# showlab/EgoVLP

Measured on AMD Instinct MI355X. Metric: clip-pairs/sec (whole node), 4f/224^2 ViT-B + 32-tok text, B=32/GPU, train step (fwd+gather+EgoNCE+bwd+AdamW), higher is better.
Workload: dtype fp16 (every Linear and both attentions of the video blocks, forward and backward) + bf16 (patch embedding, text tower, heads) MFMA operands, fp32 accumulate

## Files before the change

egovlp_amd/_lib.py:

```python
import ctypes as C
import os

import torch

_HERE = os.path.dirname(os.path.abspath(__file__))
LIB_PATH = os.environ.get("EGOVLP_HIP_LIB", os.path.join(_HERE, "libegovlp_hip.so"))

c_p = C.c_void_p
i32 = C.c_int32
i64 = C.c_int64
f32 = C.c_float
u64 = C.c_uint64


class GemmDesc(C.Structure):
    _fields_ = [
        ("a_hi", c_p), ("a_lo", c_p), ("lda", i64),
        ("b_hi", c_p), ("b_lo", c_p), ("ldb", i64),
        ("M", i32), ("N", i32), ("K", i32), ("passes", i32),
        ("alpha", f32), ("act", i32),
        ("bias", c_p),
        ("residual", c_p), ("ldr", i64),
        ("aux_in", c_p), ("aux_out", c_p), ("ldaux", i64),
        ("out_f32", c_p), ("ldo", i64),
# ... 71 lines not shown
    "egv_egonce_work_floats": (i64, [i32, i32]),
    "egv_sim_matrix_fwd": (i32, [c_p, c_p, i32, i32, i32, f32, c_p, c_p, c_p, c_p, c_p]),
    "egv_sim_matrix_bwd": (i32, [c_p, c_p, c_p, c_p, i32, i32, i32, f32, c_p, c_p, c_p]),
    "egv_egonce_from_sim": (i32, [c_p, c_p, c_p, i32, f32, i32, i32, c_p, c_p, c_p, c_p]),
    "egv_maxmargin_fwd_bwd": (i32, [c_p, c_p, i32, f32, i32, c_p, c_p, c_p]),
    "egv_maxmargin_head_fwd_bwd": (i32, [c_p, c_p, c_p, i32, i32, f32, i32, f32, c_p, c_p, c_p, c_p, c_p, c_p]),
    "egv_maxmargin_head_work_floats": (i64, [i32, i32]),
    "egv_cls_head_fwd": (i32, [c_p, i64, c_p, c_p, i32, i32, i32, c_p, i64, c_p]),
    "egv_cls_head_loss_bwd": (i32, [c_p, i64, i32, i32, i32, i32, i32, i32, c_p, i64, c_p, i32, c_p, c_p, c_p, c_p, i64, c_p, c_p, c_p]),
    "egv_cls_eval_update": (i32, [c_p, i64, i32, i32, i32, i32, i32, i32, i32, i32, c_p, c_p]),
    "egv_dual_softmax": (i32, [c_p, i32, i32, f32, c_p, c_p, c_p]),
    "egv_rank_scores": (i32, [c_p, i64, i32, c_p, i32, i64, i32, i32, i32, c_p, c_p, c_p, c_p]),
    "egv_rank_scores_work_bytes": (i64, [i32, i32]),
    "egv_cross_entropy_fwd_bwd": (i32, [c_p, i64, c_p, i32, i32, i64, c_p, c_p, i64, c_p]),
    "egv_adamw_multi": (i32, [i32, c_p, c_p, c_p, c_p, c_p, c_p, c_p, f32, f32, f32, f32, f32, i32, i32, f32, c_p, c_p]),
    "egv_grad_accumulate_multi": (i32, [i32, c_p, c_p, c_p, c_p]),
    "egv_grad_pack_bf16": (i32, [i32, c_p, c_p, c_p, c_p, f32, c_p]),
    "egv_grad_unpack_bf16": (i32, [i32, c_p, c_p, c_p, c_p, c_p]),
    "egv_slice_sum_bf16": (i32, [c_p, i32, i64, c_p, c_p]),
    "egv_relu_split": (i32, [c_p, i64, i32, i32, c_p, c_p, i64, c_p]),
    "egv_version": (i32, []),
    "egv_abi_check": (i32, [i32, i64, i64, i64, i64]),
    "egv_split_f32_multi_t16": (i32, [i32, c_p, c_p, c_p, c_p, c_p, c_p, c_p, c_p, c_p, c_p, c_p, c_p, c_p]),
    "egv_layernorm_bwd_fmt": (i32, [c_p, c_p, c_p, i64, c_p, i64, c_p, c_p, c_p, i32, i32, c_p, c_p, c_p, i64, c_p, c_p, i32, c_p, c_p, c_p, c_p]),
    "egv_layernorm_bwd_partial": (i32, [c_p, c_p, c_p, i64, c_p, i64, c_p, c_p, c_p, i32, i32, c_p, c_p, c_p, i64, c_p, c_p, i32, c_p, c_p, c_p, c_p]),
    "egv_layernorm_bwd_reduce": (i32, [i32, c_p, i32, i32, c_p, c_p, c_p]),
    "egv_splitk_reduce_multi": (i32, [i32, c_p, c_p, c_p, c_p, c_p, c_p, c_p]),
    "egv_grad_nonfinite_multi": (i32, [i32, c_p, c_p, c_p, c_p]),
    "egv_loss_scale_update": (i32, [c_p, c_p, f32, f32, f32, i32, i32, f32, f32, i32, f32, i32, c_p]),
    "egv_split_f32_multi": (i32, [i32, c_p, c_p, c_p, c_p, c_p, c_p, c_p, c_p, c_p, c_p, c_p, c_p]),
# ... 54 lines not shown
```

egovlp_amd/csrc/adamw.hip:

```cpp
#include "common.h"
#include "egovlp_hip.h"

namespace {

constexpr int MAX_T = 48;
constexpr int CHUNK = 16384;

struct AdamTable {
  float* p[MAX_T];
  const float* g[MAX_T];
  float* m[MAX_T];
  float* v[MAX_T];
  bf16_t* wh[MAX_T];
  bf16_t* wl[MAX_T];
  long numel[MAX_T];
  int blk_start[MAX_T + 1];
  int count;
};

__global__ __launch_bounds__(256) void adamw_kernel(const AdamTable t, float lr, float b1, float b2, float eps, float wd,
                                                    float step_size, float grad_scale, const float* __restrict__ hyper) {
  if (hyper) {
    if (hyper[3] != 0.f) return;
    lr = hyper[0];
    step_size = hyper[1];
    grad_scale = hyper[2];
  }
  int ti = 0;
  while (ti + 1 < t.count && (int)blockIdx.x >= t.blk_start[ti + 1]) ++ti;
  const long base = (long)((int)blockIdx.x - t.blk_start[ti]) * CHUNK;
  const long n = t.numel[ti];
  float* __restrict__ p = t.p[ti];
  const float* __restrict__ g = t.g[ti];
  float* __restrict__ m = t.m[ti];
  float* __restrict__ v = t.v[ti];
  bf16_t* wh = t.wh[ti];
  bf16_t* wl = t.wl[ti];
  const long end = min(n, base + CHUNK);
  const bool vec = ((n & 3) == 0) && (((((size_t)p) | ((size_t)g) | ((size_t)m) | ((size_t)v)) & 15) == 0) &&
                   (!wh || (((size_t)wh) & 7) == 0) && (!wl || (((size_t)wl) & 7) == 0);
  if (vec) {
    for (long i = base + threadIdx.x * 4; i < end; i += 256 * 4) {
      f32x4_t pv = egv_load<EGV_NT_ADAMW_LD, f32x4_t>(p + i), gv = egv_load<EGV_NT_ADAMW_LD, f32x4_t>(g + i),
               mv = egv_load<EGV_NT_ADAMW_LD, f32x4_t>(m + i), vv = egv_load<EGV_NT_ADAMW_LD, f32x4_t>(v + i);
      bf16_t h[4], l[4];
#pragma unroll
      for (int e = 0; e < 4; ++e) {
        const float ge = gv[e] * grad_scale;
        mv[e] = mv[e] * b1 + (1.0f - b1) * ge;
        vv[e] = vv[e] * b2 + (1.0f - b2) * ge * ge;
        const float denom = sqrtf(vv[e]) + eps;
        pv[e] = pv[e] - step_size * (mv[e] / denom);
        if (wd > 0.f) pv[e] = pv[e] - lr * wd * pv[e];
        split_bf16(pv[e], h[e], l[e]);
      }
      egv_store<EGV_NT_ADAMW_ST>(p + i, pv);
      egv_store<EGV_NT_ADAMW_ST>(m + i, mv);
      egv_store<EGV_NT_ADAMW_ST>(v + i, vv);
      if (wh) *(u32x2_t*)(wh + i) = (u32x2_t){pack2(h[0], h[1]), pack2(h[2], h[3])};
      if (wl) *(u32x2_t*)(wl + i) = (u32x2_t){pack2(l[0], l[1]), pack2(l[2], l[3])};
    }
  } else {
    for (long i = base + threadIdx.x; i < end; i += 256) {
      const float ge = g[i] * grad_scale;
      const float me = m[i] * b1 + (1.0f - b1) * ge;
      const float ve = v[i] * b2 + (1.0f - b2) * ge * ge;
      float pe = p[i] - step_size * (me / (sqrtf(ve) + eps));
      if (wd > 0.f) pe = pe - lr * wd * pe;
      p[i] = pe;
      m[i] = me;
      v[i] = ve;
      bf16_t h, l;
      split_bf16(pe, h, l);
      if (wh) wh[i] = h;
      if (wl) wl[i] = l;
    }
  }
}

constexpr int NF_MAX_T = 96;
struct NonfiniteTable {
  const float* g[NF_MAX_T];
  long numel[NF_MAX_T];
  int blk_start[NF_MAX_T + 1];
  int count;
};
__global__ __launch_bounds__(256) void grad_nonfinite_kernel(const NonfiniteTable t, int* __restrict__ state) {
  int ti = 0;
  while (ti + 1 < t.count && (int)blockIdx.x >= t.blk_start[ti + 1]) ++ti;
  const long base = (long)((int)blockIdx.x - t.blk_start[ti]) * (4 * CHUNK);
// ... 217 lines not shown
    if (!p[i] || !g[i] || !m[i] || !v[i]) return EGV_ERR_ARG;
    if (nt == MAX_T) {
      const int rc = flush();
      if (rc) return rc;
    }
    t.p[nt] = p[i]; t.g[nt] = g[i]; t.m[nt] = m[i]; t.v[nt] = v[i];
    t.wh[nt] = w_hi ? w_hi[i] : nullptr;
    t.wl[nt] = w_lo ? w_lo[i] : nullptr;
    t.numel[nt] = numel[i];
    t.blk_start[nt] = nb;
    nb += (int)((numel[i] + CHUNK - 1) / CHUNK);
    ++nt;
  }
  return flush();
}
```

egovlp_amd/csrc/gemm_nt.hip:

```cpp
#include "common.h"
#include "egovlp_hip.h"

namespace {

constexpr int BM = 128, BN = 128, BK = 32;
constexpr int PLANE_BYTES = BM * BK * 2;

struct Frag4 {
  bf16x8_t v[4];
};

__device__ __forceinline__ int swz_g(int x) { return (0x78 >> (2 * x)) & 3; }

__device__ __forceinline__ void glds16(const void* g, char* lds_wave_base) {
  __builtin_amdgcn_global_load_lds((const __attribute__((address_space(1))) void*)g,
                                   (__attribute__((address_space(3))) void*)lds_wave_base, 16, 0, 0);
}

__device__ __forceinline__ void nt_epilogue4(const egv_gemm_desc& p, f32x4_t v, int m, int n) {
  if (p.alpha != 1.0f) v *= p.alpha;
  if (p.bias) v += *(const f32x4_t*)(p.bias + n);
  if (p.act == EGV_ACT_GELU) {
    if (p.aux_out) *(f32x4_t*)(p.aux_out + (long)m * p.ldaux + n) = v;
#pragma unroll
// ... 126 lines not shown
    if (m >= p.M) continue;
#pragma unroll
    for (int j = 0; j < 4; ++j) {
      const int n = n0 + wn * 64 + j * 16 + ln;
      if (n >= p.N) continue;
      f32x4_t v = acc[i][j];
      if (ksplit > 1) {
        *(f32x4_t*)(p.partial + ((long)z * p.M + m) * p.N + n) = v;
        continue;
      }
      nt_epilogue4(p, v, m, n);
    }
  }
}

__global__ __launch_bounds__(256) void splitk_reduce_kernel(const float* __restrict__ partial, float* __restrict__ out,
                                                            long mn, int ksplit, int accumulate,
                                                            const float* __restrict__ partial2, float* __restrict__ out2,
                                                            long n2, int blocks1) {
  if ((int)blockIdx.x >= blocks1) {
    partial = partial2;
    out = out2;
    mn = n2;
    accumulate = 0;
  }
  const long i4 = ((long)((int)blockIdx.x >= blocks1 ? (int)blockIdx.x - blocks1 : (int)blockIdx.x) * blockDim.x + threadIdx.x) * 4;
  if (i4 >= mn) return;
  f32x4_t s = egv_load<EGV_NT_REDUCE_LD, f32x4_t>(partial + i4);
  for (int z = 1; z < ksplit; ++z) s += egv_load<EGV_NT_REDUCE_LD, f32x4_t>(partial + (long)z * mn + i4);
  if (accumulate) s += *(const f32x4_t*)(out + i4);
  egv_store<EGV_NT_WGRAD>(out + i4, s);
}

constexpr int RED_MAX_T = 8;
struct ReduceTable {
  const float* partial[RED_MAX_T];
  float* out[RED_MAX_T];
  float* colsum[RED_MAX_T];
  long mn[RED_MAX_T];
  int m[RED_MAX_T], ks[RED_MAX_T];
  int blk_start[RED_MAX_T + 1];
  int blocks1[RED_MAX_T];
  int count;
};
__global__ __launch_bounds__(256) void splitk_reduce_multi_kernel(const ReduceTable t) {
  int e = 0;
  while (e + 1 < t.count && (int)blockIdx.x >= t.blk_start[e + 1]) ++e;
  const int local = (int)blockIdx.x - t.blk_start[e];
  const int ks = t.ks[e];
  const float* partial = t.partial[e];
  float* out = t.out[e];
  long mn = t.mn[e];
  long i4;
  if (local >= t.blocks1[e]) {
    partial += (long)ks * mn;
    out = t.colsum[e];
    mn = t.m[e];
    i4 = ((long)(local - t.blocks1[e]) * 256 + threadIdx.x) * 4;
  } else {
    i4 = ((long)local * 256 + threadIdx.x) * 4;
  }
  if (i4 >= mn) return;
  f32x4_t s = egv_load<EGV_NT_REDUCE_LD, f32x4_t>(partial + i4);
  for (int z = 1; z < ks; ++z) s += egv_load<EGV_NT_REDUCE_LD, f32x4_t>(partial + (long)z * mn + i4);
  egv_store<EGV_NT_WGRAD>(out + i4, s);
}

}

extern "C" int egv_splitk_reduce_multi(int32_t count, const float* const* partial, float* const* out, const int64_t* mn, const int32_t* ksplit,
                                       float* const* colsum, const int32_t* m, void* stream) {
  if (count < 1 || count > RED_MAX_T || !partial || !out || !mn || !ksplit) return EGV_ERR_ARG;
  ReduceTable t = {};
  int nb = 0;
  for (int i = 0; i < count; ++i) {
    if (!partial[i] || !out[i] || mn[i] <= 0 || mn[i] % 4 != 0 || ksplit[i] < 2) return EGV_ERR_ARG;
    const bool cs = colsum && colsum[i];
    if (cs && (!m || m[i] <= 0 || m[i] % 4 != 0)) return EGV_ERR_ARG;
    t.partial[i] = partial[i]; t.out[i] = out[i]; t.colsum[i] = cs ? colsum[i] : nullptr;
    t.mn[i] = mn[i]; t.m[i] = cs ? m[i] : 0; t.ks[i] = ksplit[i];
    t.blk_start[i] = nb;
    t.blocks1[i] = (int)((mn[i] / 4 + 255) / 256);
    nb += t.blocks1[i] + (cs ? (m[i] / 4 + 255) / 256 : 0);
  }
  t.blk_start[count] = nb;
  t.count = count;
  EGV_LAUNCH(splitk_reduce_multi_kernel, dim3(nb), dim3(256), 0, (hipStream_t)stream, t);
  EGV_CHECK_LAUNCH();
  return EGV_OK;
}

int egv_gemm_big_launch(const egv_gemm_desc& p, hipStream_t s, int variant);
bool egv_gemm_big_supports(const egv_gemm_desc& p);

__global__ __launch_bounds__(256) void splitk_reduce_epilogue_kernel(const egv_gemm_desc p, int ksplit) {
  const long i4 = ((long)blockIdx.x * blockDim.x + threadIdx.x) * 4;
  const long mn = (long)p.M * p.N;
  if (i4 >= mn) return;
// ... 44 lines not shown
    EGV_LAUNCH(gemm_nt_kernel<3>, grid, block, 2 * 4 * PLANE_BYTES, s, p);
  } else {
    EGV_LAUNCH(gemm_nt_kernel<1>, grid, block, 2 * 2 * PLANE_BYTES, s, p);
  }
  EGV_CHECK_LAUNCH();
  if (ks > 1 && !p.trans && variant < 3) {
    if (p.accumulate) return EGV_ERR_ARG;
    const long mn4 = (long)p.M * p.N / 4;
    EGV_LAUNCH(splitk_reduce_epilogue_kernel, dim3((int)((mn4 + 255) / 256)), dim3(256), 0, s, p, ks);
    EGV_CHECK_LAUNCH();
  } else if (ks > 1 && p.accumulate == 2) {
    if (!p.trans || !p.out_f32 || p.ldo != p.N) return EGV_ERR_ARG;
  } else if (ks > 1) {
    if (!p.out_f32 || p.ldo != p.N) return EGV_ERR_ARG;
    const long mn = (long)p.M * p.N;
    const int blocks = (int)((mn / 4 + 255) / 256);
    if (p.colsum && p.M % 4 != 0) return EGV_ERR_ARG;
    const int blocks2 = p.colsum ? (p.M / 4 + 255) / 256 : 0;
    EGV_LAUNCH(splitk_reduce_kernel, dim3(blocks + blocks2), dim3(256), 0, s, p.partial, p.out_f32, mn, ks, p.accumulate,
               p.partial + (long)ks * mn, p.colsum, (long)p.M, blocks);
    EGV_CHECK_LAUNCH();
  }
  return EGV_OK;
}
```

egovlp_amd/ops.py:

```python
from __future__ import annotations

import contextlib
import ctypes as C
import os
import time
import sys
from dataclasses import dataclass
from typing import Optional

import torch

from . import _lib
from ._lib import GemmDesc, check

ACT_NONE, ACT_GELU, ACT_GELU_BWD, ACT_RELU_BWD = 0, 1, 2, 3


_DEFAULT_X2_BWD = os.environ.get("EGV_X2_BWD", "f16")
_AUX_BWD = int(os.environ.get("EGV_AUX_BWD", "3"))
_ENV_F16_SINGLE = os.environ.get("EGV_F16_SINGLE", "auto")
_PASSES = {"bf16x3": 3, "bf16": 1, "f16x2": 2, "f16": 4}
F16_SINGLE_BITS = {"fc1": 1, "fc2": 2, "qkv": 4, "proj": 8}
_PASSES_INV = {3: "bf16x3", 1: "bf16", 2: "f16x2", 4: "f16"}
A1_INV = 1.0 / (1.0 - 2.0 ** -6)
# ... 963 lines not shown
    arr = C.c_void_p * n
    return (arr(*[p.data_ptr() for p in params]), arr(*[m.data_ptr() for m in ms]), arr(*[v.data_ptr() for v in vs]),
            (C.c_int64 * n)(*[p.numel() for p in params]))


def adamw_multi(params, grads, ms, vs, lr, beta1, beta2, eps, weight_decay, step, correct_bias=True, grad_scale=1.0, hyper_dev=None,
                tables=None):
    n = len(params)
    P, M_, V, N = tables if tables is not None else adamw_tables(params, ms, vs)
    G = (C.c_void_p * n)(*[g.data_ptr() for g in grads])
    check(_lib.lib().egv_adamw_multi(n, P, G, M_, V, None, None, N, float(lr), float(beta1), float(beta2),
                                     float(eps), float(weight_decay), int(step), int(correct_bias),
                                     float(grad_scale), _p(hyper_dev), _stream(params[0])), "egv_adamw_multi")


class _OpsModule(type(sys.modules[__name__])):
    WGRAD_SIDE_STREAM = property(lambda m: DEFAULT.wgrad_side_stream, lambda m, v: DEFAULT.set(wgrad_side_stream=bool(v)))
    TEXT_SIDE_STREAM = property(lambda m: DEFAULT.text_side_stream, lambda m, v: DEFAULT.set(text_side_stream=bool(v)))
    BACKWARD_POLL = property(lambda m: DEFAULT.backward_poll, lambda m, v: DEFAULT.set(backward_poll=v))
    KERNEL_TIMER = property(lambda m: DEFAULT.kernel_timer, lambda m, v: DEFAULT.set(kernel_timer=v))
    GEMM_GRID = property(lambda m: DEFAULT.gemm_grid)


sys.modules[__name__].__class__ = _OpsModule
```

egovlp_amd/optim.py:

```python
import torch

from . import ops, weights


class LossScaler:

    def __init__(self, init_scale=2.0 ** 16, growth_factor=2.0, backoff_factor=0.5, growth_interval=2000, max_scale=2.0 ** 24, device="cuda"):
        if not (init_scale >= 1.0 and growth_factor >= 1.0 and 0.0 < backoff_factor <= 1.0 and growth_interval >= 1 and max_scale >= init_scale):
            raise ValueError("LossScaler: init_scale >= 1, growth_factor >= 1, 0 < backoff_factor <= 1, growth_interval >= 1, max_scale >= init_scale")
        self.growth_factor, self.backoff_factor = float(growth_factor), float(backoff_factor)
        self.growth_interval, self.max_scale = int(growth_interval), float(max_scale)
        host = torch.zeros(8, dtype=torch.int32)
        host.view(torch.float32)[0] = float(init_scale)
        host.view(torch.float32)[6] = 1.0 / float(init_scale)
        self.state = host.to(device)
        self._f = self.state.view(torch.float32)
        self.scale_tensor = self._f[0]
        self._extra_hyper = {}

    def scale(self, loss):
        return loss * self.scale_tensor

    def hyper_block(self, group_index):
        if group_index == 0:
# ... 22 lines not shown


class AdamW(torch.optim.Optimizer):
    def __init__(self, params, lr=1e-3, betas=(0.9, 0.999), eps=1e-6, weight_decay=0.0, correct_bias=True):
        if lr < 0.0:
            raise ValueError("Invalid learning rate: {} - should be >= 0.0".format(lr))
        if not 0.0 <= betas[0] < 1.0 or not 0.0 <= betas[1] < 1.0:
            raise ValueError("Invalid beta parameters: {}".format(betas))
        if not 0.0 <= eps:
            raise ValueError("Invalid epsilon value: {} - should be >= 0.0".format(eps))
        super().__init__(params, dict(lr=lr, betas=betas, eps=eps, weight_decay=weight_decay,
                                      correct_bias=correct_bias))
        self._scaler = None
        self._scaler_first = False
        self._plans = {}

    @torch.no_grad()
    def step(self, closure=None, grad_scale=1.0, scaler=None):
        loss = closure() if closure is not None else None
        groups = [(g, [p for p in g["params"] if p.grad is not None]) for g in self.param_groups]
        if scaler is not None:
            grads = [p.grad for _, ps in groups for p in ps]
            if any(g.is_sparse or not g.is_contiguous() for g in grads):
                raise RuntimeError("AdamW (HIP) needs contiguous dense gradients")
            ops.grad_nonfinite_multi(grads, scaler.state)
            self._scaler, self._scaler_first = scaler, True
        try:
            for gi, (group, params) in enumerate(groups):
                self._group_index = gi
                self._update_group(group, params, grad_scale)
        finally:
            self._scaler = None
        weights.bump_epoch()
        return loss

    def load_state_dict(self, state_dict):
        self._plans.clear()
        return super().load_state_dict(state_dict)

    def _update_group(self, group, params, grad_scale):
        plan = self._plans.get(id(group))
        if plan is not None and len(plan[0]) == len(params) and all(a is b for a, b in zip(plan[0], params)):
            _, states, ms, vs, tables, ptrs = plan
            step = states[0]["step"] + 1
            ok = all(p.data_ptr() == q for p, q in zip(params, ptrs))
            for p_, st, m, v in zip(params, states, ms, vs):
                ok = ok and st["step"] + 1 == step and st["exp_avg"] is m and st.get("exp_avg_sq") is v and self.state.get(p_) is st
                st["step"] += 1
            grads = [p.grad for p in params]
            if ok and not any(g.is_sparse or not g.is_contiguous() for g in grads):
                self._launch(group, params, grads, ms, vs, step, grad_scale, tables)
                return
            for st in states:
                st["step"] -= 1
            del self._plans[id(group)]
        ps, gs, ms, vs, sts = [], [], [], [], []
        step = None
        uniform = True
        for p in params:
            if p.grad.is_sparse:
                raise RuntimeError("AdamW does not support sparse gradients")
            st = self.state[p]
            if len(st) == 0 or "exp_avg" not in st:
                st["step"] = 0
                st["exp_avg"] = torch.zeros_like(p, memory_format=torch.contiguous_format)
                st["exp_avg_sq"] = torch.zeros_like(p, memory_format=torch.contiguous_format)
            st["step"] += 1
            if step is None:
                step = st["step"]
            elif step != st["step"]:
                self._launch(group, ps, gs, ms, vs, step, grad_scale)
                ps, gs, ms, vs, step = [], [], [], [], st["step"]
                uniform = False
            if not (p.is_contiguous() and p.grad.is_contiguous()):
                raise RuntimeError("AdamW (HIP) needs contiguous parameters and gradients")
            ps.append(p); gs.append(p.grad); ms.append(st["exp_avg"]); vs.append(st["exp_avg_sq"]); sts.append(st)
        self._launch(group, ps, gs, ms, vs, step, grad_scale)
        if uniform and ps:
            self._plans[id(group)] = (list(ps), sts, list(ms), list(vs), ops.adamw_tables(ps, ms, vs), [p.data_ptr() for p in ps])

    def _launch(self, group, ps, gs, ms, vs, step, grad_scale, tables=None):
        if not ps:
            return
        b1, b2 = group["betas"]
        hyper = None
        sc = self._scaler
        if sc is not None:
            hyper = sc.hyper_block(getattr(self, "_group_index", 0))
            ops.loss_scale_update(sc.state, hyper, group["lr"], b1, b2, step, group["correct_bias"], sc.growth_factor, sc.backoff_factor,
                                  sc.growth_interval, sc.max_scale, advance=self._scaler_first)
            self._scaler_first = False
        ops.adamw_multi(ps, gs, ms, vs, group["lr"], b1, b2, group["eps"], group["weight_decay"], step,
                        group["correct_bias"], grad_scale, hyper_dev=hyper, tables=tables)


def adamw_step_size(lr, beta1, beta2, step, correct_bias=True):
    if not correct_bias:
        return float(lr)
    import math
    return float(lr * math.sqrt(1.0 - beta2 ** step) / (1.0 - beta1 ** step))
```

egovlp_amd/trainer/common.py:

```python
from __future__ import annotations

import numpy as np
import torch

from ..base.base_trainer import Multi_BaseTrainer_dist
from ..gather import AllGather_multi


def step_prologue(model, optimizer, scaler):
    core = getattr(model, 'module', model)
    ec = getattr(core, 'exec_ctx', None)
    if scaler is None and ec is not None and ec.bwd_passes == 4:
        scaler = ec.loss_scaler(device=next(core.parameters()).device)
    optimizer.zero_grad(set_to_none=True)
    return core, ec, scaler


def step_epilogue(loss, ec, optimizer, grad_sync, scaler):
    (loss if scaler is None else scaler.scale(loss)).backward()
    if ec is not None:
        ec.join_side_stream()
    if grad_sync is not None:
        grad_sync.finish()
    if scaler is None:
        optimizer.step()
    else:
        optimizer.step(scaler=scaler)
    return loss.detach()
# ... 148 lines not shown
```

egovlp_amd/weights.py:

```python
from __future__ import annotations

import torch

from . import ops

EPOCH = 0


def bump_epoch():
    global EPOCH
    EPOCH += 1


class _Entry:
    __slots__ = ("params", "ver", "pl", "p2", "tp", "t16", "ok_token", "ok_epoch", "ok_vers")

    def __init__(self, params):
        self.params, self.ver, self.pl, self.p2, self.tp, self.t16 = params, None, None, None, None, None
        self.ok_token, self.ok_epoch, self.ok_vers = -1, -1, None

    def mark_valid(self, token):
        self.ok_token, self.ok_epoch = token, EPOCH
        self.ok_vers = [p._version for p in self.params]

# ... 75 lines not shown
                            ldt, tcols = ent.t16.ld, (ent.t16.ld - off if last else n_i)
                        jobs.append((w2, hi, lo, ldo, thi, tlo, ldt, tcols, t16))
                    if ent.p2 is not None:
                        jobs2.append((w2, ent.p2.hi.data_ptr() + off * ent.p2.ld * 2, ent.p2.lo.data_ptr() + off * ent.p2.ld * 2, ent.p2.ld))
                    off += n_i
            self._prep = (sig, ops.split_f32_multi(jobs, prepare=True), ops.f16x2_encode_multi(jobs2, prepare=True),
                          stale[0][0].params[0])
        _, run_split, run_x2, any_param = self._prep
        st = ops._stream(any_param)
        for run in (run_split, run_x2):
            if run is not None:
                run(st)
        for ent, ver in stale:
            ent.ver = ver

    def refresh(self):
        self._refresh_all()

    def begin_step(self):
        self._token += 1
        stale = self._stale(mark=True)
        self._refresh_all(stale)
        for ent, _ in stale:
            ent.mark_valid(self._token)

    def _get(self, params, need_t: bool, fmt: str = "bf16", t_fmt: str = "bf16"):
        key = id(params[0]) if len(params) == 1 else tuple(id(p) for p in params)
        ent = self._c.get(key)
        out = lambda: (ent.p2 if fmt == "f16x2" else ent.pl, ent.t16 if t_fmt == "f16" else ent.tp)
        if ent is None:
# ... 53 lines not shown
```

include/egovlp_hip.h:

```cpp
#ifndef EGOVLP_HIP_H
#define EGOVLP_HIP_H
#include <stdint.h>

#ifdef __cplusplus
extern "C" {
#endif

typedef uint16_t egv_bf16;

#define EGV_ABI_VERSION 6

enum { EGV_ACT_NONE = 0, EGV_ACT_GELU = 1, EGV_ACT_GELU_BWD = 2, EGV_ACT_RELU_BWD = 3 };

typedef struct egv_gemm_desc {
  const egv_bf16* a_hi; const egv_bf16* a_lo; int64_t lda;
  const egv_bf16* b_hi; const egv_bf16* b_lo; int64_t ldb;
  int32_t M, N, K, passes;
  float alpha;
  int32_t act;
  const float* bias;
  const float* residual; int64_t ldr;
  const float* aux_in; float* aux_out; int64_t ldaux;
  float* out_f32; int64_t ldo;
  egv_bf16* out_hi; egv_bf16* out_lo; int64_t ldoh;
// ... 183 lines not shown
#define EGV_RANK_MAX_ROW 16384
int egv_rank_scores(const float* S, int64_t lds, int32_t transposed, const void* R, int32_t r_is_f64, int64_t ldr,
                    int32_t n1, int32_t n2, int32_t affine_half, double* dcg_out, double* ap_out, void* work, void* stream);
int64_t egv_rank_scores_work_bytes(int32_t n1, int32_t n2);

int egv_grad_pack_bf16(int32_t count, const float* const* grads, const int64_t* numel, egv_bf16* flat,
                       const int64_t* offsets, float scale, void* stream);
int egv_grad_unpack_bf16(int32_t count, float* const* grads, const int64_t* numel, const egv_bf16* flat,
                         const int64_t* offsets, void* stream);
int egv_slice_sum_bf16(const egv_bf16* recv, int32_t world, int64_t slice_elems, egv_bf16* out, void* stream);

int egv_adamw_multi(int32_t count, float* const* p, const float* const* g, float* const* m, float* const* v,
                    egv_bf16* const* w_hi, egv_bf16* const* w_lo, const int64_t* numel,
                    float lr, float beta1, float beta2, float eps, float weight_decay, int32_t step,
                    int32_t correct_bias, float grad_scale, const float* hyper_dev, void* stream);
int egv_grad_accumulate_multi(int32_t count, float* const* dst, const float* const* src, const int64_t* numel, void* stream);

int egv_grad_nonfinite_multi(int32_t count, const float* const* grads, const int64_t* numel, int32_t* state, void* stream);
int egv_loss_scale_update(int32_t* state, float* hyper_out, float lr, float beta1, float beta2, int32_t step, int32_t correct_bias,
                          float growth_factor, float backoff_factor, int32_t growth_interval, float max_scale, int32_t advance,
                          void* stream);

int egv_relu_split(const float* x, int64_t ldx, int32_t rows, int32_t cols, egv_bf16* hi, egv_bf16* lo,
                   int64_t ldo, void* stream);
int egv_version(void);
int egv_abi_check(int32_t abi_version, int64_t sizeof_gemm_desc, int64_t sizeof_block_geom, int64_t sizeof_block_params,
                  int64_t sizeof_block_bwd_io);
int egv_diag_mfma_peak(int32_t iters, int32_t waves, float* out, void* stream);
int egv_diag_traffic_calib(int32_t mode, const void* src, void* dst, int64_t bytes, void* stream);

// ... 5 lines not shown
```

Baseline: 1005.

## Fuse AdamW update with weight-plane rebuild and transposes; widen split-K reduce runs

Adds an AdamW kernel that, after updating fp32 params, writes the bf16 hi/lo planes, the f16x2 planes and the transposed planes the GEMMs consume, using a shared-memory tile for the transpose. This removes the separate weight-cache refresh pass that re-read parameters after each optimizer step. The optimizer is wired to the weight cache so covered parameters are marked up to date. Split-K reduction kernels also now have each block handle a 16K-element run with unrolled loads instead of one vector per thread. The cost is more complex bookkeeping and addressing in the optimizer that must stay consistent with the cache's plane layout.

```diff
diff --git a/egovlp_amd/_lib.py b/egovlp_amd/_lib.py
--- a/egovlp_amd/_lib.py
+++ b/egovlp_amd/_lib.py
@@ -109,6 +109,7 @@
     "egv_rank_scores_work_bytes": (i64, [i32, i32]),
     "egv_cross_entropy_fwd_bwd": (i32, [c_p, i64, c_p, i32, i32, i64, c_p, c_p, i64, c_p]),
     "egv_adamw_multi": (i32, [i32, c_p, c_p, c_p, c_p, c_p, c_p, c_p, f32, f32, f32, f32, f32, i32, i32, f32, c_p, c_p]),
+    "egv_adamw_planes_multi": (i32, [i32] + [c_p] * 17 + [f32, f32, f32, f32, f32, i32, i32, f32, c_p, c_p]),
     "egv_grad_accumulate_multi": (i32, [i32, c_p, c_p, c_p, c_p]),
     "egv_grad_pack_bf16": (i32, [i32, c_p, c_p, c_p, c_p, f32, c_p]),
     "egv_grad_unpack_bf16": (i32, [i32, c_p, c_p, c_p, c_p, c_p]),
diff --git a/egovlp_amd/csrc/adamw.hip b/egovlp_amd/csrc/adamw.hip
--- a/egovlp_amd/csrc/adamw.hip
+++ b/egovlp_amd/csrc/adamw.hip
@@ -1,4 +1,5 @@
 #include "common.h"
+#include "f16x2.h"
 #include "egovlp_hip.h"
 
 namespace {
@@ -17,6 +18,16 @@
   int blk_start[MAX_T + 1];
   int count;
 };
+
+__device__ __forceinline__ void adamw_update(float& p, const float g, float& m, float& v, const float lr, const float b1, const float b2,
+                                             const float eps, const float wd, const float step_size, const float grad_scale) {
+  const float ge = g * grad_scale;
+  m = m * b1 + (1.0f - b1) * ge;
+  v = v * b2 + (1.0f - b2) * ge * ge;
+  const float denom = sqrtf(v) + eps;
+  p = p - step_size * (m / denom);
+  if (wd > 0.f) p = p - lr * wd * p;
+}
 
 __global__ __launch_bounds__(256) void adamw_kernel(const AdamTable t, float lr, float b1, float b2, float eps, float wd,
                                                     float step_size, float grad_scale, const float* __restrict__ hyper) {
@@ -46,13 +57,10 @@
       bf16_t h[4], l[4];
 #pragma unroll
       for (int e = 0; e < 4; ++e) {
-        const float ge = gv[e] * grad_scale;
-        mv[e] = mv[e] * b1 + (1.0f - b1) * ge;
-        vv[e] = vv[e] * b2 + (1.0f - b2) * ge * ge;
-        const float denom = sqrtf(vv[e]) + eps;
-        pv[e] = pv[e] - step_size * (mv[e] / denom);
-        if (wd > 0.f) pv[e] = pv[e] - lr * wd * pv[e];
-        split_bf16(pv[e], h[e], l[e]);
+        float pe = pv[e], me = mv[e], ve = vv[e];
+        adamw_update(pe, gv[e], me, ve, lr, b1, b2, eps, wd, step_size, grad_scale);
+        pv[e] = pe; mv[e] = me; vv[e] = ve;
+        split_bf16(pe, h[e], l[e]);
       }
       egv_store<EGV_NT_ADAMW_ST>(p + i, pv);
       egv_store<EGV_NT_ADAMW_ST>(m + i, mv);
@@ -62,11 +70,8 @@
     }
   } else {
     for (long i = base + threadIdx.x; i < end; i += 256) {
-      const float ge = g[i] * grad_scale;
-      const float me = m[i] * b1 + (1.0f - b1) * ge;
-      const float ve = v[i] * b2 + (1.0f - b2) * ge * ge;
-      float pe = p[i] - step_size * (me / (sqrtf(ve) + eps));
-      if (wd > 0.f) pe = pe - lr * wd * pe;
+      float pe = p[i], me = m[i], ve = v[i];
+      adamw_update(pe, g[i], me, ve, lr, b1, b2, eps, wd, step_size, grad_scale);
       p[i] = pe;
       m[i] = me;
       v[i] = ve;
@@ -74,6 +79,139 @@
       split_bf16(pe, h, l);
       if (wh) wh[i] = h;
       if (wl) wl[i] = l;
+    }
+  }
+}
+
+constexpr int PL_MAX_T = 30;
+struct AdamPlanesTable {
+  float* p[PL_MAX_T];
+  const float* g[PL_MAX_T];
+  float* m[PL_MAX_T];
+  float* v[PL_MAX_T];
+  bf16_t* hi[PL_MAX_T];
+  bf16_t* lo[PL_MAX_T];
+  bf16_t* thi[PL_MAX_T];
+  bf16_t* tlo[PL_MAX_T];
+  unsigned short* t16[PL_MAX_T];
+  unsigned short* x1[PL_MAX_T];
+  unsigned short* x2[PL_MAX_T];
+  int rows[PL_MAX_T], cols[PL_MAX_T], ldo[PL_MAX_T], ldx2[PL_MAX_T], ldt[PL_MAX_T], text[PL_MAX_T];
+  int tiles_x[PL_MAX_T];
+  int blk_start[PL_MAX_T + 1];
+  int count;
+};
+static_assert(sizeof(AdamPlanesTable) + 64 <= 4096, "the table travels in the kernel arguments");
+
+__global__ __launch_bounds__(256) void adamw_planes_kernel(const AdamPlanesTable t, float lr, float b1, float b2, float eps, float wd,
+                                                           float step_size, float grad_scale, const float* __restrict__ hyper) {
+  __shared__ float tile[64][65];
+  if (hyper) {
+    if (hyper[3] != 0.f) return;
+    lr = hyper[0];
+    step_size = hyper[1];
+    grad_scale = hyper[2];
+  }
+  int ti = 0;
+  while (ti + 1 < t.count && (int)blockIdx.x >= t.blk_start[ti + 1]) ++ti;
+  const int local = (int)blockIdx.x - t.blk_start[ti];
+  const int ty = local / t.tiles_x[ti], tx = local - ty * t.tiles_x[ti];
+  const int r0 = ty * 64, c0 = tx * 64;
+  const int rows = t.rows[ti], cols = t.cols[ti], text = t.text[ti];
+  float* __restrict__ p = t.p[ti];
+  const float* __restrict__ g = t.g[ti];
+  float* __restrict__ m = t.m[ti];
+  float* __restrict__ v = t.v[ti];
+  bf16_t* __restrict__ hi = t.hi[ti];
+  bf16_t* __restrict__ lo = t.lo[ti];
+  unsigned short* __restrict__ x1 = t.x1[ti];
+  unsigned short* __restrict__ x2 = t.x2[ti];
+  bf16_t* __restrict__ thi = t.thi[ti];
+  bf16_t* __restrict__ tlo = t.tlo[ti];
+  unsigned short* __restrict__ t16 = t.t16[ti];
+  const long ldo = t.ldo[ti], ldx2 = t.ldx2[ti], ldt = t.ldt[ti];
+  const bool has_t = thi || t16;
+  const int tid = threadIdx.x;
+  const int tr = tid >> 3;
+  const int tc = (tid & 7) * 8;
+#pragma unroll
+  for (int rr = 0; rr < 64; rr += 32) {
+    const int r = r0 + rr + tr, c = c0 + tc;
+    float w[8] = {0.f, 0.f, 0.f, 0.f, 0.f, 0.f, 0.f, 0.f};
+    const bool in0 = r < rows && c < cols, in1 = r < rows && c + 4 < cols;
+    if (in0) {
+      const long o = (long)r * cols + c;
+      f32x4_t pv[2], gv[2], mv[2], vv[2];
+#pragma unroll
+      for (int h = 0; h < 2; ++h) {
+        if (h == 0 || in1) {
+          pv[h] = egv_load<EGV_NT_ADAMW_LD, f32x4_t>(p + o + 4 * h);
+          gv[h] = egv_load<EGV_NT_ADAMW_LD, f32x4_t>(g + o + 4 * h);
+          mv[h] = egv_load<EGV_NT_ADAMW_LD, f32x4_t>(m + o + 4 * h);
+          vv[h] = egv_load<EGV_NT_ADAMW_LD, f32x4_t>(v + o + 4 * h);
+        }
+      }
+#pragma unroll
+      for (int h = 0; h < 2; ++h) {
+        if (h == 0 || in1) {
+#pragma unroll
+          for (int e = 0; e < 4; ++e) {
+            float pe = pv[h][e], me = mv[h][e], ve = vv[h][e];
+            adamw_update(pe, gv[h][e], me, ve, lr, b1, b2, eps, wd, step_size, grad_scale);
+            pv[h][e] = pe; mv[h][e] = me; vv[h][e] = ve;
+            w[4 * h + e] = pe;
+          }
+          egv_store<EGV_NT_ADAMW_ST>(p + o + 4 * h, pv[h]);
+          egv_store<EGV_NT_ADAMW_ST>(m + o + 4 * h, mv[h]);
+          egv_store<EGV_NT_ADAMW_ST>(v + o + 4 * h, vv[h]);
+        }
+      }
+      if (hi) {
+        bf16_t bh[8], bl[8];
+#pragma unroll
+        for (int e = 0; e < 8; ++e) split_bf16(w[e], bh[e], bl[e]);
+        const u32x4_t ph = {pack2(bh[0], bh[1]), pack2(bh[2], bh[3]), pack2(bh[4], bh[5]), pack2(bh[6], bh[7])};
+        const u32x4_t pq = {pack2(bl[0], bl[1]), pack2(bl[2], bl[3]), pack2(bl[4], bl[5]), pack2(bl[6], bl[7])};
+        if (in1) {
+          *(u32x4_t*)(hi + (long)r * ldo + c) = ph;
+          if (lo) *(u32x4_t*)(lo + (long)r * ldo + c) = pq;
+        } else {
+          *(u32x2_t*)(hi + (long)r * ldo + c) = (u32x2_t){ph[0], ph[1]};
+          if (lo) *(u32x2_t*)(lo + (long)r * ldo + c) = (u32x2_t){pq[0], pq[1]};
+        }
+      }
+      if (x1) {
+        u32x4_t o1, o2;
+        f16x2_encode8<1>(w, o1, o2);
+        *(u32x4_t*)(x1 + (long)r * ldx2 + c) = o1;
+        *(u32x4_t*)(x2 + (long)r * ldx2 + c) = o2;
+      }
+    }
+    if (has_t) {
+#pragma unroll
+      for (int e = 0; e < 8; ++e) tile[rr + tr][tc + e] = w[e];
+    }
+  }
+  if (!has_t) return;
+  __syncthreads();
+  const int ur = tid >> 4;
+  const int uc = (tid & 15) * 4;
+#pragma unroll
+  for (int cc = 0; cc < 64; cc += 16) {
+    const int c = c0 + cc + ur, r = r0 + uc;
+    if (c < cols && r < text) {
+      float x[4];
+#pragma unroll
+      for (int e = 0; e < 4; ++e) x[e] = (r + e < rows) ? tile[uc + e][cc + ur] : 0.f;
+      if (t16)
+        *(u32x2_t*)(t16 + (long)c * ldt + r) = (u32x2_t){f16_pk(f16x2_clamp(x[0]), f16x2_clamp(x[1])), f16_pk(f16x2_clamp(x[2]), f16x2_clamp(x[3]))};
+      if (thi) {
+        bf16_t bh[4], bl[4];
+#pragma unroll
+        for (int e = 0; e < 4; ++e) split_bf16(x[e], bh[e], bl[e]);
+        *(u32x2_t*)(thi + (long)c * ldt + r) = (u32x2_t){pack2(bh[0], bh[1]), pack2(bh[2], bh[3])};
+        if (tlo) *(u32x2_t*)(tlo + (long)c * ldt + r) = (u32x2_t){pack2(bl[0], bl[1]), pack2(bl[2], bl[3])};
+      }
     }
   }
 }
@@ -321,3 +459,69 @@
   }
   return flush();
 }
+
+extern "C" int egv_adamw_planes_multi(int32_t count, float* const* p, const float* const* g, float* const* m, float* const* v,
+                                      const int32_t* rows, const int32_t* cols, egv_bf16* const* pl_hi, egv_bf16* const* pl_lo,
+                                      const int64_t* ld_pl, egv_bf16* const* tp_hi, egv_bf16* const* tp_lo, uint16_t* const* t16,
+                                      const int64_t* ldt, const int32_t* t_cols, uint16_t* const* p2_hi, uint16_t* const* p2_lo,
+                                      const int64_t* ld_p2, float lr, float beta1, float beta2, float eps, float weight_decay,
+                                      int32_t step, int32_t correct_bias, float grad_scale, const float* hyper_dev, void* stream) {
+  if (count < 0 || !p || !g || !m || !v || !rows || !cols || !pl_hi || !pl_lo || !ld_pl || !tp_hi || !tp_lo || !t16 || !ldt || !t_cols ||
+      !p2_hi || !p2_lo || !ld_p2 || step < 1)
+    return EGV_ERR_ARG;
+  auto misaligned = [](const void* q, size_t a) { return (((size_t)q) & (a - 1)) != 0; };
+  for (int i = 0; i < count; ++i) {
+    if (!p[i] || !g[i] || !m[i] || !v[i] || rows[i] <= 0 || cols[i] <= 0 || cols[i] % 4 != 0) return EGV_ERR_ARG;
+    if (misaligned(p[i], 16) || misaligned(g[i], 16) || misaligned(m[i], 16) || misaligned(v[i], 16)) return EGV_ERR_ARG;
+    if (pl_lo[i] && !pl_hi[i]) return EGV_ERR_ARG;
+    if (pl_hi[i] && (ld_pl[i] < cols[i] || ld_pl[i] % 8 != 0 || ld_pl[i] > 0x7fffffff || misaligned(pl_hi[i], 16) || misaligned(pl_lo[i], 16)))
+      return EGV_ERR_ARG;
+    if ((p2_hi[i] != nullptr) != (p2_lo[i] != nullptr)) return EGV_ERR_ARG;
+    if (p2_hi[i] && (cols[i] % 8 != 0 || ld_p2[i] < cols[i] || ld_p2[i] % 8 != 0 || ld_p2[i] > 0x7fffffff || misaligned(p2_hi[i], 16) ||
+                     misaligned(p2_lo[i], 16)))
+      return EGV_ERR_ARG;
+    if (tp_lo[i] && !tp_hi[i]) return EGV_ERR_ARG;
+    if ((tp_hi[i] || t16[i]) &&
+        (ldt[i] < rows[i] || ldt[i] % 4 != 0 || ldt[i] > 0x7fffffff || t_cols[i] < rows[i] || t_cols[i] > ldt[i] || t_cols[i] % 4 != 0 ||
+         misaligned(tp_hi[i], 8) || misaligned(tp_lo[i], 8) || misaligned(t16[i], 8)))
+      return EGV_ERR_ARG;
+  }
+  float step_size = lr;
+  if (correct_bias) {
+    const double bc1 = 1.0 - pow((double)beta1, (double)step);
+    const double bc2 = 1.0 - pow((double)beta2, (double)step);
+    step_size = (float)((double)lr * sqrt(bc2) / bc1);
+  }
+  hipStream_t s = (hipStream_t)stream;
+  AdamPlanesTable t;
+  int nt = 0, nb = 0;
+  auto flush = [&]() -> int {
+    if (nt == 0) return EGV_OK;
+    t.blk_start[nt] = nb;
+    t.count = nt;
+    EGV_LAUNCH(adamw_planes_kernel, dim3(nb), dim3(256), 0, s, t, lr, beta1, beta2, eps, weight_decay, step_size, grad_scale, hyper_dev);
+    EGV_CHECK_LAUNCH();
+    nt = 0;
+    nb = 0;
+    return EGV_OK;
+  };
+  for (int i = 0; i < count; ++i) {
+    if (nt == PL_MAX_T) {
+      const int rc = flush();
+      if (rc) return rc;
+    }
+    const bool has_t = tp_hi[i] || t16[i];
+    const int row_extent = has_t ? t_cols[i] : rows[i];
+    const int tx = (cols[i] + 63) / 64, ty = (row_extent + 63) / 64;
+    t.p[nt] = p[i]; t.g[nt] = g[i]; t.m[nt] = m[i]; t.v[nt] = v[i];
+    t.hi[nt] = pl_hi[i]; t.lo[nt] = pl_lo[i]; t.thi[nt] = tp_hi[i]; t.tlo[nt] = tp_lo[i]; t.t16[nt] = t16[i];
+    t.x1[nt] = p2_hi[i]; t.x2[nt] = p2_lo[i];
+    t.rows[nt] = rows[i]; t.cols[nt] = cols[i]; t.ldo[nt] = (int)ld_pl[i]; t.ldx2[nt] = (int)ld_p2[i]; t.ldt[nt] = (int)ldt[i];
+    t.text[nt] = has_t ? t_cols[i] : rows[i];
+    t.tiles_x[nt] = tx;
+    t.blk_start[nt] = nb;
+    nb += tx * ty;
+    ++nt;
+  }
+  return flush();
+}
diff --git a/egovlp_amd/csrc/gemm_nt.hip b/egovlp_amd/csrc/gemm_nt.hip
--- a/egovlp_amd/csrc/gemm_nt.hip
+++ b/egovlp_amd/csrc/gemm_nt.hip
@@ -164,22 +164,64 @@
   }
 }
 
+constexpr int RED_RUN = 16384;
+__device__ __forceinline__ void splitk_reduce_run(const float* __restrict__ partial, float* __restrict__ out, long mn, int ks, long base,
+                                                  int accumulate) {
+  const long end = min(mn, base + RED_RUN);
+  long i = base + threadIdx.x * 4;
+  for (; i + 3 * 1024 < end; i += 4 * 1024) {
+    f32x4_t s[4];
+#pragma unroll
+    for (int u = 0; u < 4; ++u) s[u] = egv_load<EGV_NT_REDUCE_LD, f32x4_t>(partial + i + u * 1024);
+    int z = 1;
+    for (; z + 1 < ks; z += 2) {
+      f32x4_t a[4], b[4];
+#pragma unroll
+      for (int u = 0; u < 4; ++u) {
+        a[u] = egv_load<EGV_NT_REDUCE_LD, f32x4_t>(partial + (long)z * mn + i + u * 1024);
+        b[u] = egv_load<EGV_NT_REDUCE_LD, f32x4_t>(partial + (long)(z + 1) * mn + i + u * 1024);
+      }
+#pragma unroll
+      for (int u = 0; u < 4; ++u) {
+        s[u] += a[u];
+        s[u] += b[u];
+      }
+    }
+    if (z < ks) {
+#pragma unroll
+      for (int u = 0; u < 4; ++u) s[u] += egv_load<EGV_NT_REDUCE_LD, f32x4_t>(partial + (long)z * mn + i + u * 1024);
+    }
+    if (accumulate) {
+#pragma unroll
+      for (int u = 0; u < 4; ++u) s[u] += *(const f32x4_t*)(out + i + u * 1024);
+    }
+#pragma unroll
+    for (int u = 0; u < 4; ++u) egv_store<EGV_NT_WGRAD>(out + i + u * 1024, s[u]);
+  }
+  for (; i < end; i += 1024) {
+    f32x4_t s = egv_load<EGV_NT_REDUCE_LD, f32x4_t>(partial + i);
+    int z = 1;
+    for (; z + 3 < ks; z += 4) {
+      f32x4_t a[4];
+#pragma unroll
+      for (int u = 0; u < 4; ++u) a[u] = egv_load<EGV_NT_REDUCE_LD, f32x4_t>(partial + (long)(z + u) * mn + i);
+#pragma unroll
+      for (int u = 0; u < 4; ++u) s += a[u];
+    }
+    for (; z < ks; ++z) s += egv_load<EGV_NT_REDUCE_LD, f32x4_t>(partial + (long)z * mn + i);
+    if (accumulate) s += *(const f32x4_t*)(out + i);
+    egv_store<EGV_NT_WGRAD>(out + i, s);
+  }
+}
+
 __global__ __launch_bounds__(256) void splitk_reduce_kernel(const float* __restrict__ partial, float* __restrict__ out,
                                                             long mn, int ksplit, int accumulate,
                                                             const float* __restrict__ partial2, float* __restrict__ out2,
                                                             long n2, int blocks1) {
-  if ((int)blockIdx.x >= blocks1) {
-    partial = partial2;
-    out = out2;
-    mn = n2;
-    accumulate = 0;
-  }
-  const long i4 = ((long)((int)blockIdx.x >= blocks1 ? (int)blockIdx.x - blocks1 : (int)blockIdx.x) * blockDim.x + threadIdx.x) * 4;
-  if (i4 >= mn) return;
-  f32x4_t s = egv_load<EGV_NT_REDUCE_LD, f32x4_t>(partial + i4);
-  for (int z = 1; z < ksplit; ++z) s += egv_load<EGV_NT_REDUCE_LD, f32x4_t>(partial + (long)z * mn + i4);
-  if (accumulate) s += *(const f32x4_t*)(out + i4);
-  egv_store<EGV_NT_WGRAD>(out + i4, s);
+  if ((int)blockIdx.x >= blocks1)
+    splitk_reduce_run(partial2, out2, n2, ksplit, (long)((int)blockIdx.x - blocks1) * RED_RUN, 0);
+  else
+    splitk_reduce_run(partial, out, mn, ksplit, (long)blockIdx.x * RED_RUN, accumulate);
 }
 
 constexpr int RED_MAX_T = 8;
@@ -198,22 +240,11 @@
   while (e + 1 < t.count && (int)blockIdx.x >= t.blk_start[e + 1]) ++e;
   const int local = (int)blockIdx.x - t.blk_start[e];
   const int ks = t.ks[e];
-  const float* partial = t.partial[e];
-  float* out = t.out[e];
-  long mn = t.mn[e];
-  long i4;
-  if (local >= t.blocks1[e]) {
-    partial += (long)ks * mn;
-    out = t.colsum[e];
-    mn = t.m[e];
-    i4 = ((long)(local - t.blocks1[e]) * 256 + threadIdx.x) * 4;
-  } else {
-    i4 = ((long)local * 256 + threadIdx.x) * 4;
-  }
-  if (i4 >= mn) return;
-  f32x4_t s = egv_load<EGV_NT_REDUCE_LD, f32x4_t>(partial + i4);
-  for (int z = 1; z < ks; ++z) s += egv_load<EGV_NT_REDUCE_LD, f32x4_t>(partial + (long)z * mn + i4);
-  egv_store<EGV_NT_WGRAD>(out + i4, s);
+  const long mn = t.mn[e];
+  if (local >= t.blocks1[e])
+    splitk_reduce_run(t.partial[e] + (long)ks * mn, t.colsum[e], (long)t.m[e], ks, (long)(local - t.blocks1[e]) * RED_RUN, 0);
+  else
+    splitk_reduce_run(t.partial[e], t.out[e], mn, ks, (long)local * RED_RUN, 0);
 }
 
 }
@@ -230,8 +261,8 @@
     t.partial[i] = partial[i]; t.out[i] = out[i]; t.colsum[i] = cs ? colsum[i] : nullptr;
     t.mn[i] = mn[i]; t.m[i] = cs ? m[i] : 0; t.ks[i] = ksplit[i];
     t.blk_start[i] = nb;
-    t.blocks1[i] = (int)((mn[i] / 4 + 255) / 256);
-    nb += t.blocks1[i] + (cs ? (m[i] / 4 + 255) / 256 : 0);
+    t.blocks1[i] = (int)((mn[i] + RED_RUN - 1) / RED_RUN);
+    nb += t.blocks1[i] + (cs ? (m[i] + RED_RUN - 1) / RED_RUN : 0);
   }
   t.blk_start[count] = nb;
   t.count = count;
@@ -306,9 +337,9 @@
   } else if (ks > 1) {
     if (!p.out_f32 || p.ldo != p.N) return EGV_ERR_ARG;
     const long mn = (long)p.M * p.N;
-    const int blocks = (int)((mn / 4 + 255) / 256);
+    const int blocks = (int)((mn + RED_RUN - 1) / RED_RUN);
     if (p.colsum && p.M % 4 != 0) return EGV_ERR_ARG;
-    const int blocks2 = p.colsum ? (p.M / 4 + 255) / 256 : 0;
+    const int blocks2 = p.colsum ? (p.M + RED_RUN - 1) / RED_RUN : 0;
     EGV_LAUNCH(splitk_reduce_kernel, dim3(blocks + blocks2), dim3(256), 0, s, p.partial, p.out_f32, mn, ks, p.accumulate,
                p.partial + (long)ks * mn, p.colsum, (long)p.M, blocks);
     EGV_CHECK_LAUNCH();
diff --git a/egovlp_amd/ops.py b/egovlp_amd/ops.py
--- a/egovlp_amd/ops.py
+++ b/egovlp_amd/ops.py
@@ -1001,6 +1001,29 @@
                                      float(grad_scale), _p(hyper_dev), _stream(params[0])), "egv_adamw_multi")
 
 
+_ADAMW_PLANES = int(os.environ.get("EGV_ADAMW_PLANES", "1"))
+
+
+def adamw_planes_tables(jobs, ms, vs):
+    n = len(jobs)
+    vp, i64, i32 = C.c_void_p * n, C.c_int64 * n, C.c_int32 * n
+    col = lambda k: [j[k] or None for j in jobs]
+    return (vp(*[j[0].data_ptr() for j in jobs]), vp(*[m.data_ptr() for m in ms]), vp(*[v.data_ptr() for v in vs]),
+            i32(*[j[1] for j in jobs]), i32(*[j[2] for j in jobs]), vp(*col(3)), vp(*col(4)), i64(*[j[5] for j in jobs]),
+            vp(*col(6)), vp(*col(7)), vp(*col(8)), i64(*[j[9] for j in jobs]), i32(*[j[10] for j in jobs]),
+            vp(*col(11)), vp(*col(12)), i64(*[j[13] for j in jobs]))
+
+
+def adamw_planes_multi(params, grads, tables, lr, beta1, beta2, eps, weight_decay, step, correct_bias=True, grad_scale=1.0,
+                       hyper_dev=None):
+    n = len(params)
+    P, M_, V, R, Cc, HI, LO, LDO, THI, TLO, T16, LDT, TC, X1, X2, LDX = tables
+    G = (C.c_void_p * n)(*[g.data_ptr() for g in grads])
+    check(_lib.lib().egv_adamw_planes_multi(n, P, G, M_, V, R, Cc, HI, LO, LDO, THI, TLO, T16, LDT, TC, X1, X2, LDX, float(lr),
+                                            float(beta1), float(beta2), float(eps), float(weight_decay), int(step), int(correct_bias),
+                                            float(grad_scale), _p(hyper_dev), _stream(params[0])), "egv_adamw_planes_multi")
+
+
 class _OpsModule(type(sys.modules[__name__])):
     WGRAD_SIDE_STREAM = property(lambda m: DEFAULT.wgrad_side_stream, lambda m, v: DEFAULT.set(wgrad_side_stream=bool(v)))
     TEXT_SIDE_STREAM = property(lambda m: DEFAULT.text_side_stream, lambda m, v: DEFAULT.set(text_side_stream=bool(v)))
diff --git a/egovlp_amd/optim.py b/egovlp_amd/optim.py
--- a/egovlp_amd/optim.py
+++ b/egovlp_amd/optim.py
@@ -60,6 +60,14 @@
         self._scaler = None
         self._scaler_first = False
         self._plans = {}
+        self._plane_cache = None
+        self._plane_plans = {}
+        self._written = []
+
+    def attach_plane_cache(self, cache):
+        if cache is not self._plane_cache:
+            self._plane_cache = cache
+            self._plane_plans.clear()
 
     @torch.no_grad()
     def step(self, closure=None, grad_scale=1.0, scaler=None):
@@ -77,11 +85,17 @@
                 self._update_group(group, params, grad_scale)
         finally:
             self._scaler = None
+            written, self._written = self._written, []
+        if scaler is not None:
+            written = [ent for ent in written if ent.ver == ent.version()]
         weights.bump_epoch()
+        if written:
+            self._plane_cache.mark_updated(written)
         return loss
 
     def load_state_dict(self, state_dict):
         self._plans.clear()
+        self._plane_plans.clear()
         return super().load_state_dict(state_dict)
 
     def _update_group(self, group, params, grad_scale):
@@ -95,11 +109,21 @@
                 st["step"] += 1
             grads = [p.grad for p in params]
             if ok and not any(g.is_sparse or not g.is_contiguous() for g in grads):
-                self._launch(group, params, grads, ms, vs, step, grad_scale, tables)
+                pp = self._plane_plan(group, params, ms, vs)
+                if pp is None or any(grads[i].data_ptr() % 16 for i in pp[1]):
+                    self._launch(group, params, grads, ms, vs, step, grad_scale, tables)
+                else:
+                    _, idx, ptab, ents, rest, rtab = pp
+                    hyper = self._hyper(group, step)
+                    self._launch(group, [params[i] for i in rest], [grads[i] for i in rest], None, None, step, grad_scale, rtab, hyper=hyper)
+                    self._launch(group, [params[i] for i in idx], [grads[i] for i in idx], None, None, step, grad_scale, ptab, hyper=hyper,
+                                 planes=True)
+                    self._written.extend(ents)
                 return
             for st in states:
                 st["step"] -= 1
             del self._plans[id(group)]
+            self._plane_plans.pop(id(group), None)
         ps, gs, ms, vs, sts = [], [], [], [], []
         step = None
         uniform = True
@@ -122,20 +146,50 @@
                 raise RuntimeError("AdamW (HIP) needs contiguous parameters and gradients")
             ps.append(p); gs.append(p.grad); ms.append(st["exp_avg"]); vs.append(st["exp_avg_sq"]); sts.append(st)
         self._launch(group, ps, gs, ms, vs, step, grad_scale)
+        self._plane_plans.pop(id(group), None)
         if uniform and ps:
             self._plans[id(group)] = (list(ps), sts, list(ms), list(vs), ops.adamw_tables(ps, ms, vs), [p.data_ptr() for p in ps])
 
-    def _launch(self, group, ps, gs, ms, vs, step, grad_scale, tables=None):
+    def _plane_plan(self, group, params, ms, vs):
+        wc = self._plane_cache
+        if wc is None or not ops._ADAMW_PLANES:
+            return None
+        sig = wc.update_signature()
+        pp = self._plane_plans.get(id(group))
+        if pp is None or pp[0] != sig:
+            ents, jobs = wc.update_jobs(params)
+            where = {id(p): i for i, p in enumerate(params)}
+            idx = [where[id(j[0])] for j in jobs]
+            if len(set(idx)) != len(idx):
+                ents, jobs, idx = [], [], []
+            taken = set(idx)
+            rest = [i for i in range(len(params)) if i not in taken]
+            pp = (sig, idx, ops.adamw_planes_tables(jobs, [ms[i] for i in idx], [vs[i] for i in idx]) if idx else None, ents, rest,
+                  ops.adamw_tables([params[i] for i in rest], [ms[i] for i in rest], [vs[i] for i in rest]))
+            self._plane_plans[id(group)] = pp
+        return pp if pp[1] else None
+
+    def _hyper(self, group, step):
+        sc = self._scaler
+        if sc is None:
+            return None
+        b1, b2 = group["betas"]
+        hyper = sc.hyper_block(getattr(self, "_group_index", 0))
+        ops.loss_scale_update(sc.state, hyper, group["lr"], b1, b2, step, group["correct_bias"], sc.growth_factor, sc.backoff_factor,
+                              sc.growth_interval, sc.max_scale, advance=self._scaler_first)
+        self._scaler_first = False
+        return hyper
+
+    def _launch(self, group, ps, gs, ms, vs, step, grad_scale, tables=None, hyper=False, planes=False):
         if not ps:
             return
         b1, b2 = group["betas"]
-        hyper = None
-        sc = self._scaler
-        if sc is not None:
-            hyper = sc.hyper_block(getattr(self, "_group_index", 0))
-            ops.loss_scale_update(sc.state, hyper, group["lr"], b1, b2, step, group["correct_bias"], sc.growth_factor, sc.backoff_factor,
-                                  sc.growth_interval, sc.max_scale, advance=self._scaler_first)
-            self._scaler_first = False
+        if hyper is False:
+            hyper = self._hyper(group, step)
+        if planes:
+            ops.adamw_planes_multi(ps, gs, tables, group["lr"], b1, b2, group["eps"], group["weight_decay"], step,
+                                   group["correct_bias"], grad_scale, hyper_dev=hyper)
+            return
         ops.adamw_multi(ps, gs, ms, vs, group["lr"], b1, b2, group["eps"], group["weight_decay"], step,
                         group["correct_bias"], grad_scale, hyper_dev=hyper, tables=tables)
 
diff --git a/egovlp_amd/trainer/common.py b/egovlp_amd/trainer/common.py
--- a/egovlp_amd/trainer/common.py
+++ b/egovlp_amd/trainer/common.py
@@ -12,6 +12,9 @@
     ec = getattr(core, 'exec_ctx', None)
     if scaler is None and ec is not None and ec.bwd_passes == 4:
         scaler = ec.loss_scaler(device=next(core.parameters()).device)
+    attach = getattr(optimizer, 'attach_plane_cache', None)
+    if attach is not None and ec is not None:
+        attach(ec.wc)
     optimizer.zero_grad(set_to_none=True)
     return core, ec, scaler
 
diff --git a/egovlp_amd/weights.py b/egovlp_amd/weights.py
--- a/egovlp_amd/weights.py
+++ b/egovlp_amd/weights.py
@@ -113,6 +113,60 @@
         for ent, ver in stale:
             ent.ver = ver
 
+    @staticmethod
+    def _addresses(ent):
+        def at(pl):
+            return 0 if pl is None else (pl.hi.data_ptr(), pl.lo.data_ptr() if pl.lo is not None else 0)
+        return (at(ent.pl), at(ent.tp), at(ent.p2), at(ent.t16), tuple(p.data_ptr() for p in ent.params))
+
+    def update_signature(self):
+        return tuple((id(ent),) + self._addresses(ent) for ent in self._c.values())
+
+    def update_jobs(self, params):
+        ids = {id(p) for p in params}
+        ents, jobs = [], []
+        for ent in self._c.values():
+            if not all(id(p) in ids for p in ent.params) or not ent.shapes_ok():
+                continue
+            off, mine = 0, []
+            for i, p in enumerate(ent.params):
+                n_i = p.shape[0] if p.dim() >= 2 else 0
+                k = p[0].numel() if n_i else 0
+                if (n_i == 0 or p.dtype != torch.float32 or not p.is_contiguous() or p.data_ptr() % 16 or k % 4
+                        or (ent.p2 is not None and k % 8) or off % 4):
+                    mine = None
+                    break
+                last = i == len(ent.params) - 1
+                hi = lo = thi = tlo = t16 = x1 = x2 = 0
+                ldo = ldt = ldx = 0
+                tcols = n_i
+                if ent.pl is not None:
+                    ldo = ent.pl.ld
+                    hi, lo = ent.pl.hi.data_ptr() + off * ldo * 2, ent.pl.lo.data_ptr() + off * ldo * 2
+                if ent.tp is not None:
+                    ldt, tcols = ent.tp.ld, (ent.tp.ld - off if last else n_i)
+                    thi, tlo = ent.tp.hi.data_ptr() + off * 2, ent.tp.lo.data_ptr() + off * 2
+                if ent.t16 is not None:
+                    ldt, tcols = ent.t16.ld, (ent.t16.ld - off if last else n_i)
+                    t16 = ent.t16.hi.data_ptr() + off * 2
+                if ent.p2 is not None:
+                    ldx = ent.p2.ld
+                    x1, x2 = ent.p2.hi.data_ptr() + off * ldx * 2, ent.p2.lo.data_ptr() + off * ldx * 2
+                if ldo % 8 or ldx % 8 or (hi | lo | x1 | x2) % 16 or (thi | tlo | t16) % 8 or tcols % 4:
+                    mine = None
+                    break
+                mine.append((p, n_i, k, hi, lo, ldo, thi, tlo, t16, ldt, tcols, x1, x2, ldx))
+                off += n_i
+            if mine:
+                ents.append(ent)
+                jobs.extend(mine)
+        return ents, jobs
+
+    @staticmethod
+    def mark_updated(ents):
+        for ent in ents:
+            ent.ver = ent.version()
+
     def refresh(self):
         self._refresh_all()
 
diff --git a/include/egovlp_hip.h b/include/egovlp_hip.h
--- a/include/egovlp_hip.h
+++ b/include/egovlp_hip.h
@@ -221,6 +221,12 @@
                     egv_bf16* const* w_hi, egv_bf16* const* w_lo, const int64_t* numel,
                     float lr, float beta1, float beta2, float eps, float weight_decay, int32_t step,
                     int32_t correct_bias, float grad_scale, const float* hyper_dev, void* stream);
+int egv_adamw_planes_multi(int32_t count, float* const* p, const float* const* g, float* const* m, float* const* v,
+                           const int32_t* rows, const int32_t* cols, egv_bf16* const* pl_hi, egv_bf16* const* pl_lo,
+                           const int64_t* ld_pl, egv_bf16* const* tp_hi, egv_bf16* const* tp_lo, uint16_t* const* t16,
+                           const int64_t* ldt, const int32_t* t_cols, uint16_t* const* p2_hi, uint16_t* const* p2_lo,
+                           const int64_t* ld_p2, float lr, float beta1, float beta2, float eps, float weight_decay, int32_t step,
+                           int32_t correct_bias, float grad_scale, const float* hyper_dev, void* stream);
 int egv_grad_accumulate_multi(int32_t count, float* const* dst, const float* const* src, const int64_t* numel, void* stream);
 
 int egv_grad_nonfinite_multi(int32_t count, const float* const* grads, const int64_t* numel, int32_t* state, void* stream);
```

New measurement: 1012 (median of 6 runs). Within noise of the previous version (+0.7%).
